# RIKEN-RCCS/EigenExa

Hardware: AMD Instinct MI355X
Metric: eigen_sx full-solve throughput (reference flop model: 4/3 N^3 + D&C GEMM + 2 nvec N^2) (higher is better)
Workload: dtype f64; 1 GPU; N=8192 random symmetric fp64 (counter-based R+R^T, seed 20240807), eigen_sx all eigenpairs, m_forward=64, m_backward=128; parallelism=1 GPU (1x1 grid)

## Files before the change

eigenexa_amd/csrc/api.hip:

```cpp
#include "eigx_context.h"
#include "eigx_comm.h"
#include "../../include/eigenexa_amd.h"
#include <cstring>

namespace eigx {
Context g_ctx;
}

using namespace eigx;

extern "C" {

int eigx_init(int device) {
  return eigx_init_multi(device, 0, 1, nullptr, 'C');
}

int eigx_get_device_count(void) {
  int ndev = 0;
  if (hipGetDeviceCount(&ndev) != hipSuccess) { (void)hipGetLastError(); return 0; }
  return ndev;
}

int eigx_get_rccl_unique_id(void* out128) {
  return comm_get_unique_id(out128);
// ... 15 lines not shown
  int ndev = 0;
  if (hipGetDeviceCount(&ndev) != hipSuccess || ndev <= 0) {
    fprintf(stderr, "[eigx] no HIP device visible: this library has no CPU path\n");
    return EIGX_ERR_NO_DEVICE;
  }
  if (device < 0 || device >= ndev) return EIGX_ERR_BAD_ARG;
  EIGX_HIP_CHECK(hipSetDevice(device));
  g_ctx.device = device;
  int Px = 1;
  for (int x = 1; x * x <= nranks; ++x)
    if (nranks % x == 0) Px = x;
  int req_px = 0, req_py = 0;
  if (g_next_px > 0) {
    const int rx = g_next_px, ry = g_next_py;
    req_px = rx; req_py = ry;
    g_next_px = g_next_py = 0;
    if (rx * ry != nranks) {
      fprintf(stderr, "[eigx] illegal grid dimensions %d x %d for %d ranks\n", rx, ry, nranks);
      return EIGX_ERR_BAD_ARG;
    }
    Px = rx;
  }
  Grid g;
  g.Px = Px;
  g.Py = nranks / Px;
  g.rank = rank;
  g.nranks = nranks;
  if (order == 'R' || order == 'r') {
    g.px = rank / g.Py;
    g.py = rank % g.Py;
    g.row_major = 1;
  } else {
    g.px = rank % g.Px;
    g.py = rank / g.Px;
    g.row_major = 0;
  }
  g_ctx.grid = g;
  if (nranks > 1) {
    const int rc = comm_init(g_ctx, uid);
    if (rc != 0) {
      g_ctx.grid = Grid();
      g_next_px = req_px; g_next_py = req_py;
      return rc;
    }
  }
  EIGX_HIP_CHECK(hipStreamCreateWithFlags(&g_ctx.stream, hipStreamNonBlocking));
  EIGX_HIP_CHECK(hipStreamCreateWithFlags(&g_ctx.side_stream, hipStreamNonBlocking));
  for (int q = 0; q < Context::kAux; ++q)
    EIGX_HIP_CHECK(hipStreamCreateWithFlags(&g_ctx.aux[q], hipStreamNonBlocking));
  for (int q = 0; q <= Context::kAux; ++q)
    EIGX_HIP_CHECK(hipEventCreateWithFlags(&g_ctx.aux_ev[q], hipEventDisableTiming));
  EIGX_HIP_CHECK(hipEventCreateWithFlags(&g_ctx.bt_ev, hipEventDisableTiming));
  EIGX_HIP_CHECK(hipEventCreateWithFlags(&g_ctx.dc_ev, hipEventDisableTiming));
  {
    int prio_lo = 0, prio_hi = 0;
    EIGX_HIP_CHECK(hipDeviceGetStreamPriorityRange(&prio_lo, &prio_hi));
    EIGX_HIP_CHECK(hipStreamCreateWithPriority(&g_ctx.dc_stream, hipStreamNonBlocking, prio_hi));
  }
  EIGX_HIP_CHECK(hipEventCreateWithFlags(&g_ctx.dc_b_ev, hipEventDisableTiming));
  EIGX_HIP_CHECK(hipEventCreateWithFlags(&g_ctx.dc_z_ev, hipEventDisableTiming));
  g_ctx.bt_stream = g_ctx.side_stream;
  g_ctx.initialized = true;
  g_ctx.errinfo = 0;
  return EIGX_OK;
}

int eigx_free(void) {
  if (!g_ctx.initialized) return EIGX_OK;
  EIGX_HIP_CHECK(hipSetDevice(g_ctx.device));
  EIGX_HIP_CHECK(hipDeviceSynchronize());
  if (g_ctx.grid.nranks > 1) comm_free(g_ctx);
  g_ctx.pool.release();
  for (hipEvent_t e : g_ctx.prof_ev) EIGX_HIP_CHECK(hipEventDestroy(e));
  EIGX_HIP_CHECK(hipStreamDestroy(g_ctx.stream));
  EIGX_HIP_CHECK(hipStreamDestroy(g_ctx.side_stream));
  for (int q = 0; q < Context::kAux; ++q) EIGX_HIP_CHECK(hipStreamDestroy(g_ctx.aux[q]));
  for (int q = 0; q <= Context::kAux; ++q) EIGX_HIP_CHECK(hipEventDestroy(g_ctx.aux_ev[q]));
  EIGX_HIP_CHECK(hipEventDestroy(g_ctx.bt_ev));
  EIGX_HIP_CHECK(hipEventDestroy(g_ctx.dc_ev));
  EIGX_HIP_CHECK(hipStreamDestroy(g_ctx.dc_stream));
  g_ctx.bt_stream = nullptr;
  EIGX_HIP_CHECK(hipEventDestroy(g_ctx.dc_b_ev));
  EIGX_HIP_CHECK(hipEventDestroy(g_ctx.dc_z_ev));
  g_ctx = Context();
  return EIGX_OK;
}

int eigx_get_version(int* version, char* date32, char* vcode32) {
  if (version) *version = 10;
  if (date32) { memset(date32, 0, 32); strncpy(date32, "2026-10", 31); }
  if (vcode32) { memset(vcode32, 0, 32); strncpy(vcode32, "eigenexa_amd gfx950", 31); }
  return EIGX_OK;
}

int eigx_get_procs(int* procs, int* x_procs, int* y_procs) {
  if (!g_ctx.initialized) return EIGX_ERR_NOT_INITIALIZED;
  if (procs) *procs = g_ctx.grid.nranks;
  if (x_procs) *x_procs = g_ctx.grid.Px;
  if (y_procs) *y_procs = g_ctx.grid.Py;
  return EIGX_OK;
}

int eigx_get_id(int* id, int* x_id, int* y_id) {
  if (!g_ctx.initialized) return EIGX_ERR_NOT_INITIALIZED;
  if (id) *id = g_ctx.grid.rank + 1;
  if (x_id) *x_id = g_ctx.grid.px + 1;
  if (y_id) *y_id = g_ctx.grid.py + 1;
  return EIGX_OK;
}

int eigx_get_comm(int* x_color, int* x_key, int* y_color, int* y_key) {
  if (!g_ctx.initialized) return EIGX_ERR_NOT_INITIALIZED;
  const Grid& g = g_ctx.grid;
  if (x_color) *x_color = g.py + 1;
  if (x_key) *x_key = g.px + 1;
  if (y_color) *y_color = g.px + 1;
  if (y_key) *y_key = g.py + 1;
  return EIGX_OK;
}

double eigx_comm_seconds(void) { return g_ctx.timers[4]; }

int eigx_comm_info(char* buf, int len) {
  if (!g_ctx.initialized) return EIGX_ERR_NOT_INITIALIZED;
  return comm_info(g_ctx, buf, len);
}

int eigx_get_errinfo(int64_t* info) {
  if (info) *info = g_ctx.errinfo;
  return EIGX_OK;
}

// ... 128 lines not shown
    out[3 * k + 1] += g_ctx.prof_units[q];
    out[3 * k + 2] += 1e-3 * ms;
  }
  return EIGX_OK;
}

int eigx_device_synchronize(void) {
  if (!g_ctx.initialized) return EIGX_ERR_NOT_INITIALIZED;
  EIGX_HIP_CHECK(hipSetDevice(g_ctx.device));
  EIGX_HIP_CHECK(hipDeviceSynchronize());
  return EIGX_OK;
}

void* eigx_malloc_dev(int64_t bytes) {
  if (!g_ctx.initialized) return nullptr;
  void* p = nullptr;
  if (hipMalloc(&p, (size_t)bytes) != hipSuccess) return nullptr;
  return p;
}
int eigx_free_dev(void* p) {
  if (p) EIGX_HIP_CHECK(hipFree(p));
  return EIGX_OK;
}
int eigx_memcpy_h2d(void* dst, const void* src, int64_t bytes) {
  EIGX_HIP_CHECK(hipMemcpy(dst, src, (size_t)bytes, hipMemcpyHostToDevice));
  return EIGX_OK;
}
int eigx_memcpy_d2h(void* dst, const void* src, int64_t bytes) {
  EIGX_HIP_CHECK(hipMemcpy(dst, src, (size_t)bytes, hipMemcpyDeviceToHost));
  return EIGX_OK;
}

int eigx_tune(int key, int value) {
  if (key == 0) return set_gemm_variant(value);
  if (key == 1) return set_bisect_threads(value);
  if (key == 2) return set_bt_q(value);
  if (key == 3 || key == 4 || key == 5 || key == 10 || key == 11) return set_reduce_knob(key, value);
  if (key == 12) return (value >= 0 && value <= 2) ? set_reduce_knob(key, value) : -1;
  if (key == 6) return set_gemm_cstream(value);
  if (key == 7) return value > 0 ? set_reduce_knob(key, value) : -1;
  if (key == 8) return set_dc_chunk(value);
  if (key == 9) return comm_set_bounce(value);
  if (key == 15) return set_dc_pipe(value);
  if (key == 16) return set_dc_batch(value);
  if (key == 17 || key == 18 || key == 19) return set_range_knob(key, value);
  if (key == 20) return set_tri_nb(value);
  if (key == 21) return set_batch_nmax(value);
  if (key == 22) return set_hbatch_nmax(value);
  if (key == 23) return set_gbatch_nmax(value);
  if (key == 24) return set_hgbatch_nmax(value);
  if (key == 25) return set_gemm_latec_kmax(value);
  if (key == 26) return set_batch_range_route(value);
  if (key == 27) return set_batch_range_accept(value);
  return -1;
}

int eigx_dgemm_dev(char opa, char opb, int m, int n, int k, double alpha, const double* a, int lda,
                   const double* b, int ldb, double beta, double* c, int ldc, int tri_upper) {
  if (!g_ctx.initialized) return EIGX_ERR_NOT_INITIALIZED;
  EIGX_HIP_CHECK(hipStreamSynchronize(nullptr));
  dgemm_dev(g_ctx.stream, opa, opb, m, n, k, alpha, a, lda, b, ldb, beta, c, ldc, tri_upper ? 1 : 0,
            &g_ctx.grid);
  EIGX_HIP_CHECK(hipStreamSynchronize(g_ctx.stream));
  return EIGX_OK;
}

int eigx_dgemm_gather_dev(char opa, char opb, int m, int n, int k, double alpha, const double* a, int lda,
                          const double* b, int ldb, double beta, double* c, int ldc, const int* kmap_a,
                          const int* kmap_b) {
  if (!g_ctx.initialized) return EIGX_ERR_NOT_INITIALIZED;
  EIGX_HIP_CHECK(hipStreamSynchronize(nullptr));
  dgemm_dev(g_ctx.stream, opa, opb, m, n, k, alpha, a, lda, b, ldb, beta, c, ldc, 0, nullptr, kmap_a, nullptr, 1, 0,
            0, 0, 1, 0, 0, 0, 1, 0, kmap_b);
  EIGX_HIP_CHECK(hipStreamSynchronize(g_ctx.stream));
  return EIGX_OK;
}

}
```

eigenexa_amd/csrc/band_reduce.hip:

```cpp
#include "eigx_context.h"
#include "eigx_comm.h"
#include "../../include/eigenexa_amd.h"
#include <algorithm>
#include <chrono>
#include <cstring>
#include <type_traits>

#pragma clang fp contract(on)

namespace eigx {

namespace {

static inline int pd_rows_for(int toprows) { int r = ((toprows + 3) / 4 + 63) / 64 * 64; return r < 512 ? 512 : r; }
#ifdef EIGX_STAMPS
#define EIGX_ABL(bit) (R.abl & (bit))
#define EIGX_STAMP(slot) do { if (R.dbg && threadIdx.x == 0 && stamp_me) { \
  const unsigned long long _t = __builtin_amdgcn_s_memtime(); atomicAdd(&R.dbg[slot], _t - stamp_prev); stamp_prev = _t; } } while (0)
#define EIGX_STAMP_INIT const bool stamp_me = (bid == nblocks / 2); unsigned long long stamp_prev = __builtin_amdgcn_s_memtime(); (void)stamp_me;
#else
#define EIGX_ABL(bit) false
#define EIGX_STAMP(slot) do {} while (0)
#define EIGX_STAMP_INIT
#endif
constexpr int PD_COLS = 16;
constexpr int KA_ROWS = 16;
constexpr int KA_SL = 256 / KA_ROWS;

enum { SC_SA = 0, SC_BETA_A = 1, SC_SB = 2, SC_BETA_B = 3, SC_COUNT = 8 };

struct RedArgs {
  double* A; int lda; int n;
  double* UW; int ldp; int m;
  double* X;
  double* YR; double* YC;
  double* KD;
  double* SP;
  int sp_packed;
  int kd_compact;
  double* GP;
  double* sc;
  double* d; double* e; int lde;
  int maxseg, maxrs, maxchunk, gp2_off, kdab_off;
  int P, me;
  float invP;
  int Px, Py, px, py, row_major;
  int nxs, nys;
  const double* MSG;
  int msg_stride;
  size_t ypar_stride; int ysrc_stride;
  const double* XW;
  int xmsg_stride, nown;
  size_t xpar_stride;
  const double* PAN; int ldpan;
  const double* zero16;
  int abl;
  int stamp_i;
  unsigned long long* dbg;
};

struct SymvGeom { int L, T, nt; };

int g_ka_fit = 1;
int g_ka_loads = 2;
int g_ka_wgs = 256;
int g_symv_t128 = 4500, g_symv_t256 = 40000;
int g_symv_nt = 9000;
int g_symv_unc = 9000;
}

int set_reduce_knob(int key, int v) {
  int* t = key == 3 ? &g_symv_t128 : key == 4 ? &g_symv_t256 : key == 5 ? &g_symv_nt : key == 7 ? &g_ka_wgs
         : key == 10 ? &g_ka_fit : key == 11 ? &g_symv_unc : key == 12 ? &g_ka_loads : nullptr;
  if (!t) return -1;
  const int old = *t;
  *t = v;
  return old;
}

namespace {

inline SymvGeom symv_geom(int L) {
  SymvGeom g;
  g.L = L;
  g.T = (L <= g_symv_t128) ? 128 : (L <= g_symv_t256 ? 256 : 512);
  g.nt = (L + g.T - 1) / g.T;
  return g;
}

typedef double d2v_t __attribute__((ext_vector_type(2)));
template <bool NT>
__device__ __forceinline__ double2 ld2(const double* p) {
  const d2v_t v = NT ? __builtin_nontemporal_load(reinterpret_cast<const d2v_t*>(p)) : *reinterpret_cast<const d2v_t*>(p);
  return make_double2(v.x, v.y);
}

template <int CTRL>
__device__ __forceinline__ double dpp_add(double v) {
  const int lo = __double2loint(v), hi = __double2hiint(v);
  const int lo2 = __builtin_amdgcn_update_dpp(0, lo, CTRL, 0xf, 0xf, true);
  const int hi2 = __builtin_amdgcn_update_dpp(0, hi, CTRL, 0xf, 0xf, true);
  return v + __hiloint2double(hi2, lo2);
}

template <int CTRL>
__device__ __forceinline__ double dpp_mov(double v) {
  const int lo2 = __builtin_amdgcn_update_dpp(0, __double2loint(v), CTRL, 0xf, 0xf, true);
  const int hi2 = __builtin_amdgcn_update_dpp(0, __double2hiint(v), CTRL, 0xf, 0xf, true);
  return __hiloint2double(hi2, lo2);
}

__device__ __forceinline__ double swapadd32(double a, double b) {
  const auto lo = __builtin_amdgcn_permlane32_swap(__double2loint(a), __double2loint(b), false, false);
  const auto hi = __builtin_amdgcn_permlane32_swap(__double2hiint(a), __double2hiint(b), false, false);
  return __hiloint2double(hi[0], lo[0]) + __hiloint2double(hi[1], lo[1]);
}
__device__ __forceinline__ double swapadd16(double a, double b) {
  const auto lo = __builtin_amdgcn_permlane16_swap(__double2loint(a), __double2loint(b), false, false);
  const auto hi = __builtin_amdgcn_permlane16_swap(__double2hiint(a), __double2hiint(b), false, false);
  return __hiloint2double(hi[0], lo[0]) + __hiloint2double(hi[1], lo[1]);
}

__device__ __forceinline__ double wave_sum(double v) {
  v = dpp_add<0xB1>(v);
  v = dpp_add<0x4E>(v);
  v = dpp_add<0x141>(v);
  v = dpp_add<0x140>(v);
// ... 1464 lines not shown
__global__ void compact_panel_kernel(const double* __restrict__ UW, int ldp, int m, int nrl, int ncl, int Px, int px,
                                     int Py, int py, double* __restrict__ UWr, int ldr, double* __restrict__ UWc, int ldc) {
  const int k = blockIdx.y;
  const double* rsrc = UW + (size_t)k * ldp;
  const double* csrc = UW + (size_t)(k + m) * ldp;
  for (int l = blockIdx.x * blockDim.x + threadIdx.x; l < (nrl > ncl ? nrl : ncl); l += gridDim.x * blockDim.x) {
    if (l < nrl) UWr[(size_t)k * ldr + l] = rsrc[(size_t)l * Px + px];
    if (l < ncl) UWc[(size_t)k * ldc + l] = csrc[(size_t)l * Py + py];
  }
}

__global__ void pack_panel_kernel(const double* __restrict__ A, int lda, int lj0, int mloc, int nrl, int nxs,
                                  double* __restrict__ send) {
  const int ljr = blockIdx.y;
  if (ljr >= mloc) return;
  for (int li = blockIdx.x * blockDim.x + threadIdx.x; li < nrl; li += gridDim.x * blockDim.x)
    send[(size_t)ljr * nxs + li] = A[(size_t)(lj0 + ljr) * lda + li];
}
__global__ void unpack_panel_kernel(const double* __restrict__ recv, size_t count, int nxs, int clo, int chi, int toprows,
                                    int Px, int Py, int row_major, double* __restrict__ PAN, int ldpan) {
  const int c = clo + blockIdx.y;
  if (c > chi) return;
  const int qy = c % Py;
  const int lj0 = (clo - qy + Py - 1) / Py;
  const int ljr = c / Py - lj0;
  for (int r = blockIdx.x * blockDim.x + threadIdx.x; r < toprows; r += gridDim.x * blockDim.x) {
    const int qx = r % Px;
    const int src = row_major ? qx * Py + qy : qx + qy * Px;
    PAN[(size_t)(c - clo) * ldpan + r] = ld_sys(recv + (size_t)src * count + (size_t)ljr * nxs + r / Px);
  }
}

template <int NB>
__global__ void mg_wcopy_kernel(RedArgs R, int xpar, int wk, int rows, StepWait W) {
  if (W.n > 0) step_wait_fused(W, blockIdx.x == 0);
  double* Wp = R.UW + (size_t)R.ldp * R.m;
  for (int r = blockIdx.x * blockDim.x + threadIdx.x; r < rows; r += gridDim.x * blockDim.x) {
    int s_, o_;
    own_of(R, r, s_, o_);
    const double* xm = R.XW + (size_t)xpar * R.xpar_stride + (size_t)s_ * R.xmsg_stride + o_;
    Wp[(size_t)wk * R.ldp + r] = ld_sys(xm + 2 * (size_t)R.nown);
    if (NB == 2) Wp[(size_t)(wk + 1) * R.ldp + r] = ld_sys(xm + 3 * (size_t)R.nown);
  }
}
template <int NB>
__global__ void mg_tail_kernel(RedArgs R, int xpar, int i, int ncols, StepWait W) {
  if (W.n > 0) step_wait_fused(W, blockIdx.x == 0);
  if (threadIdx.x == 0 && ncols > 0) {
    R.d[i] = xget<true>(R, xpar, 0, i);
    if (ncols > 1) { R.e[i] = xget<true>(R, xpar, 0, i - 1); R.d[i - 1] = xget<true>(R, xpar, 1, i - 1); }
  }
}

inline double wall_seconds() { return std::chrono::duration<double>(std::chrono::steady_clock::now().time_since_epoch()).count(); }
inline StepWait no_wait() { return StepWait{nullptr, nullptr, nullptr, 0, 0, 0, 1}; }
inline void clear_panel(const RedArgs& R, hipStream_t st) {
  hipLaunchKernelGGL(fill_kernel, dim3(1024), dim3(256), 0, st, R.UW, (size_t)R.ldp * R.m * 3, 0.0);
}

template <int NB>
RedArgs reduce_setup(Context& ctx, int n, double* A, int lda, double* d, double* e, int lde, int m) {
  m = std::min(std::max(m, NB), 256);
  if (NB == 2 && (m & 1)) ++m;
  const int ldp = pad_ld((n + 127) / 128 * 128 + 128);
  const Grid& G = ctx.grid;
  const bool mg = G.nranks > 1;
  RedArgs R;
  R.A = A; R.lda = lda; R.n = n; R.ldp = ldp; R.m = m;
  R.d = d; R.e = e; R.lde = lde;
  R.P = G.nranks; R.me = G.rank; R.invP = 1.0f / (float)G.nranks;
  R.Px = G.Px; R.Py = G.Py; R.px = G.px; R.py = G.py; R.row_major = G.row_major;
  R.nxs = (ceil_div(n, G.Px) + 7) / 8 * 8; R.nys = (ceil_div(n, G.Py) + 7) / 8 * 8;
  R.msg_stride = NB * (R.nxs + R.nys) + 8 + 2 * NB * m;
  R.ypar_stride = (size_t)G.nranks * R.msg_stride; R.ysrc_stride = R.msg_stride;
  R.nown = ceil_div(ceil_div(n, KA_ROWS), G.nranks) * KA_ROWS;
  R.xmsg_stride = 4 * R.nown + 8;
  R.xpar_stride = (size_t)G.nranks * R.xmsg_stride;
  R.MSG = nullptr; R.XW = nullptr; R.PAN = nullptr; R.ldpan = ldp;
  int maxseg = 0;
  if (mg) maxseg = ceil_div(R.nxs > R.nys ? R.nxs : R.nys, 128) + 1;
  else for (int L = n; L >= 1; --L) maxseg = std::max(maxseg, symv_geom(L).nt);
  maxseg += 1;
  R.maxseg = maxseg; R.maxrs = maxseg; R.maxchunk = 4 + 1;
  R.UW = ctx.pool.get_t<double>("red.UW", (size_t)ldp * (m * 3 + 128));
  R.X = ctx.pool.get_t<double>("red.X", (size_t)ldp * 3);
  if (!mg) {
    const int nslot = (maxseg + 2 > 162) ? maxseg + 2 : 162;
    R.YC = ctx.pool.get_t<double>("red.Y", (size_t)nslot * NB * ldp);
    R.YR = R.YC + (size_t)NB * ldp;
    R.kdab_off = R.maxchunk * 2 * NB * m;
    R.KD = ctx.pool.get_t<double>("red.KD", (size_t)R.kdab_off + R.maxchunk + 8 + 512);
  } else {
    R.YR = ctx.pool.get_t<double>("red.YR", (size_t)maxseg * NB * ldp);
    R.YC = ctx.pool.get_t<double>("red.YC", (size_t)R.maxrs * NB * ldp);
    const int maxchunk2 = 12;
    R.kdab_off = maxchunk2 * 2 * NB * m;
    R.KD = ctx.pool.get_t<double>("red.KD2", (size_t)R.kdab_off + 4 * G.nranks + 4 + 8 + 512);
  }
  R.SP = ctx.pool.get_t<double>("red.SP", (size_t)(maxseg * maxseg) * 3 + 8);
  R.sp_packed = (!mg && g_ka_loads >= 1) ? 1 : 0;
  R.kd_compact = (!mg && g_ka_loads >= 2) ? 1 : 0;
  R.gp2_off = 0;
  R.GP = ctx.pool.get_t<double>("red.GP", (size_t)((n + KA_ROWS - 1) / KA_ROWS + 2) * 3 + 8);
  R.sc = ctx.pool.get_t<double>("red.sc", SC_COUNT + 8);
  R.zero16 = R.sc + SC_COUNT;
  R.dbg = nullptr; R.abl = 0; R.stamp_i = -1;
#ifdef EIGX_STAMPS
  R.abl = getenv("EIGX_ABL") ? atoi(getenv("EIGX_ABL")) : 0;
  R.stamp_i = getenv("EIGX_STAMP_I") ? atoi(getenv("EIGX_STAMP_I")) : -1;
  R.dbg = ctx.pool.get_t<unsigned long long>("red.dbg", 4096);
  EIGX_HIP_CHECK(hipMemsetAsync(R.dbg, 0, 4096 * sizeof(unsigned long long), ctx.stream));
#endif
  clear_panel(R, ctx.stream);
  hipLaunchKernelGGL(fill_kernel, dim3(8), dim3(256), 0, ctx.stream, e, (size_t)lde * NB, 0.0);
  hipLaunchKernelGGL(fill_kernel, dim3(1), dim3(64), 0, ctx.stream, R.sc, (size_t)SC_COUNT + 8, 0.0);
  hipLaunchKernelGGL(fill_kernel, dim3(16), dim3(256), 0, ctx.stream, R.SP, (size_t)(maxseg * maxseg) * 3 + 8, 0.0);
  return R;
}

struct RedCounters {
  long n_symv = 0, n_k1 = 0; double symv_bytes = 0.0, k1_flops = 0.0;
  bool sampled(const Context& ctx) const { return ctx.prof_stride > 0 && (n_symv % ctx.prof_stride) == 0; }
  void step(int L) { symv_bytes += 8.0 * ((double)L * (L + 1) / 2); ++n_symv; }
  void panel(int nr, int m) { k1_flops += 2.0 * (double)nr * nr * m; ++n_k1; }
  void write(Context& ctx) const { ctx.timers[6] = (double)n_k1; ctx.timers[7] = k1_flops; ctx.timers[9] = (double)n_symv; ctx.timers[10] = symv_bytes; }
};
inline KAArgs ka_first_args() { KAArgs S{}; S.lgT_prev = 7; S.G = 1; S.wait = no_wait(); return S; }
template <int NB>
inline int ka_step_args(KAArgs& S, int i, int k) {
  const int L = i - NB + 1;
  S.ncols = (L >= 1) ? NB : (i >= 0 ? (i + 1 < NB ? i + 1 : NB) : 0);
  S.i = i; S.L = (L >= 1) ? L : 0; S.k = k;
  S.rows = (S.has_prev && S.iprev + 1 > i + 1) ? S.iprev + 1 : i + 1;
  return L;
}
template <int NB>
inline void step_done(KAArgs& S, RedCounters& C, int& i, int& k, int L, int nt, int T, int nchunk, int nchunk_ab) {
  C.step(L);
  S.has_prev = 1; S.iprev = i; S.Lprev = L; S.kprev = k; S.nchunk_prev = nchunk; S.nchunk_ab = nchunk_ab;
  S.nt_prev = nt; S.lgT_prev = (T == 128) ? 7 : (T == 256 ? 8 : 9);
  k += NB;
  i -= NB;
}
template <int NB>
inline bool panel_full(int k, int m, int i) { return k >= m && i - NB + 1 >= 1; }
inline void panel_restart(const RedArgs& R, RedCounters& C, KAArgs& S, int& k, int nr, hipStream_t st) {
  C.panel(nr, R.m); clear_panel(R, st); S.has_prev = 0; k = 0;
}
inline KAArgs ka_close_args(const KAArgs& S, int i, int k) { KAArgs F = S; F.ncols = 0; F.i = i; F.L = 0; F.k = k; F.rows = S.iprev + 1; return F; }
inline KBArgs kb_step_args(int i, int L, int k) {
  KBArgs B;
  B.i = i; B.L = L; B.k = k;
  B.ncg = (k + PD_COLS - 1) / PD_COLS; B.toprows = i + 1; B.pdr = pd_rows_for(B.toprows);
  B.nown_L = 0; B.npd_s = 0; B.pdr_s = 0; B.wk = -1; B.xpar = 0; B.xwait = no_wait();
  B.Lr = L; B.Lc = L; B.ntc = 0; B.nty_last = 0; B.slope = 0; B.c1 = 0;
  return B;
}
inline void trace_enqueue(double t_begin, hipStream_t st) {
  if (!getenv("EIGX_TRACE_ENQUEUE")) return;
  const double te = wall_seconds();
  EIGX_HIP_CHECK(hipStreamSynchronize(st));
  fprintf(stderr, "[eigx] reduction: enqueue loop %.1f ms, then %.1f ms until the stream drained\n", (te - t_begin) * 1e3, (wall_seconds() - te) * 1e3);
}
inline void stamps_report(const RedArgs& R, int NB, hipStream_t st) {
#ifdef EIGX_STAMPS
  const bool mg = R.P > 1;
// ... 49 lines not shown
    auto go_kb = [&](auto kb, auto pwc) {
      constexpr int RPB = decltype(rpb)::value, SPB = decltype(spb)::value, KB = decltype(kb)::value, PW = decltype(pwc)::value;
      constexpr bool SPK = decltype(spk)::value;
      if (K.G > 1) hipLaunchKernelGGL((ka_kernel<NB, false, true, RPB, SPB, KB, PW, SPK>), dim3(nwg), dim3(256), 0, st, R, K);
      else hipLaunchKernelGGL((ka_kernel<NB, false, false, RPB, SPB, KB, PW, SPK>), dim3(nwg), dim3(256), 0, st, R, K);
    };
    auto go_pw = [&](auto kb) {
      if constexpr (decltype(spk)::value) {
        if constexpr (decltype(kb)::value <= 4) {
          if (pw == 1) return go_kb(kb, IC<1>{});
        }
        if (pw == 2) return go_kb(kb, IC<2>{});
      }
      go_kb(kb, IC<0>{});
    };
    if (kk <= 2 * KA_SL) go_pw(IC<2>{}); else if (kk <= 4 * KA_SL) go_pw(IC<4>{}); else go_pw(IC<8>{});
  };
  if (R.sp_packed) {
    const std::true_type pk{};
    if (nslot <= 1 * KA_SL && ntl <= 256) go(IC<1>{}, IC<1>{}, pk);
    else if (nslot <= 2 * KA_SL && ntl <= 256) go(IC<2>{}, IC<1>{}, pk);
    else if (nslot <= 2 * KA_SL && ntl <= 512) go(IC<2>{}, IC<2>{}, pk);
    else if (nslot <= 3 * KA_SL && ntl <= 768) go(IC<3>{}, IC<3>{}, pk);
    else if (nslot <= 3 * KA_SL && ntl <= 1024) go(IC<3>{}, IC<4>{}, pk);
    else if (nslot <= 3 * KA_SL) go(IC<3>{}, IC<8>{}, pk);
    else if (nslot <= 5 * KA_SL) go(IC<5>{}, IC<8>{}, pk);
    else go(IC<10>{}, IC<8>{}, pk);
    return;
  }
  const std::false_type fl{};
  if (nslot <= 1 * KA_SL && ntp <= 15) go(IC<1>{}, IC<2>{}, fl);
  else if (nslot <= 2 * KA_SL && ntp <= 31) go(IC<2>{}, IC<4>{}, fl);
  else if (nslot <= 3 * KA_SL) go(IC<3>{}, IC<8>{}, fl);
  else if (nslot <= 5 * KA_SL) go(IC<5>{}, IC<8>{}, fl);
  else go(IC<10>{}, IC<8>{}, fl);
}

template <class Go>
void symv_variant(int T, bool nt_loads, bool unc, Go&& go) {
  auto u = [&](auto rb, auto ntl) { if (unc) go(rb, ntl, std::true_type{}); else go(rb, ntl, std::false_type{}); };
  if (T == 128) u(IC<1>{}, std::false_type{});
  else if (T == 256 && !nt_loads) u(IC<2>{}, std::false_type{});
  else if (T == 256) u(IC<2>{}, std::true_type{});
  else if (!nt_loads) u(IC<4>{}, std::false_type{});
  else u(IC<4>{}, std::true_type{});
}
template <int NB>
void launch_symv(hipStream_t st, int gx, const RedArgs& R, const KBArgs& B, int T, bool nt_loads, bool unc) {
  symv_variant(T, nt_loads, unc, [&](auto rb, auto ntl, auto un) {
    hipLaunchKernelGGL((symv_kernel<NB, decltype(rb)::value, decltype(ntl)::value, false, decltype(un)::value>), dim3(gx), dim3(256), 0, st, R, B);
  });
}

template <int NB>
void reduce_one_gpu(Context& ctx, const RedArgs& R, RedCounters& C) {
  const hipStream_t st = ctx.stream;
  const int m = R.m, ldp = R.ldp;
  const double t_begin = wall_seconds();
  KAArgs S = ka_first_args();
  int k = 0, i = R.n - 1;
  while (true) {
    const int L = ka_step_args<NB>(S, i, k);
    const int nb_ka = ka_grid_one_gpu(S.rows, S.G);
    if (S.rows > 0 && (S.has_prev || S.ncols > 0)) launch_ka<NB>(st, nb_ka, R, S);
    if (L < 1) break;
    KBArgs B = kb_step_args(i, L, k);
    const SymvGeom g = symv_geom(L);
    B.npd = (B.toprows + B.pdr - 1) / B.pdr; B.ngp = nb_ka; B.nt = g.nt; B.ng = g.T / 32;
    const int gx = g.nt * (g.nt + 1) / 2 + B.npd * (B.ncg + 1);
    const bool prof = C.sampled(ctx);
    if (prof) ctx.prof_begin(0, 8.0 * ((double)L * (L + 1) / 2), st);
    launch_symv<NB>(st, gx, R, B, g.T, L > g_symv_nt, L <= g_symv_unc);
    if (prof) ctx.prof_end(st);
    step_done<NB>(S, C, i, k, L, g.nt, g.T, B.npd, B.npd);
    if (panel_full<NB>(k, m, i)) {
      KAArgs F = ka_close_args(S, i, k);
      const int nb_kf = ka_grid_one_gpu(F.rows, F.G);
      launch_ka<NB>(st, nb_kf, R, F);
      const int nr = i + 1;
      if (ctx.prof_stride > 0) ctx.prof_begin(1, 2.0 * (double)nr * nr * m, st);
      dgemm_dev(st, 'N', 'T', nr, nr, 2 * m, -1.0, R.UW, ldp, R.UW + (size_t)ldp * m, ldp, 1.0, R.A, R.lda, 1);
      if (ctx.prof_stride > 0) ctx.prof_end(st);
      panel_restart(R, C, S, k, nr, st);
    }
  }
  trace_enqueue(t_begin, st);
}

template <int NB>
void launch_mg_step(hipStream_t st, int gx, const RedArgs& R, const KLArgs& KL, const KAArgs& S, const KBArgs& B,
                    const MGStep& M, int symv_T, bool nt_loads, bool unc) {
  if (symv_T == 0) hipLaunchKernelGGL((mg_step_kernel<NB, 1, false, true>), dim3(gx), dim3(256), 0, st, R, KL, S, B, M);
  else symv_variant(symv_T, nt_loads, unc, [&](auto rb, auto ntl, auto un) {
    hipLaunchKernelGGL((mg_step_kernel<NB, decltype(rb)::value, decltype(ntl)::value, decltype(un)::value>), dim3(gx), dim3(256), 0, st,
                       R, KL, S, B, M);
  });
}

inline int mg_step_geom(KBArgs& B, const Grid& G, int L, int& ntiles) {
  const int gfull = L / KA_ROWS, rem = L % KA_ROWS;
  B.nown_L = local_count(gfull, G.nranks, G.rank) * KA_ROWS + ((rem > 0 && gfull % G.nranks == G.rank) ? rem : 0);
  B.pdr = std::max(512, ((B.nown_L + 7) / 8 + 63) / 64 * 64);
  B.npd = (B.nown_L + B.pdr - 1) / B.pdr;
  B.pdr_s = std::max(512, ((B.toprows + 4 * G.nranks - 1) / (4 * G.nranks) + 63) / 64 * 64);
  B.npd_s = (B.toprows + B.pdr_s - 1) / B.pdr_s;
  B.ngp = G.nranks;
  B.Lr = local_count(L, G.Px, G.px); B.Lc = local_count(L, G.Py, G.py);
  const double leq = sqrt((double)(B.Lr > 1 ? B.Lr : 1) * (double)(B.Lc > 1 ? B.Lc : 1));
  const int T = (leq <= g_symv_t128) ? 128 : (leq <= g_symv_t256 ? 256 : 512);
  B.ntc = B.nt = ceil_div(B.Lc, T); B.ng = T / 32;
  ntiles = B.nty_last = B.ntc > 0 ? mg_nty(B.ntc - 1, T, B.Lc, G.Px, G.px, G.Py, G.py) : 0;
  for (int tx = 0; tx + 1 < B.ntc; ++tx) ntiles += mg_nty(tx, T, B.Lc, G.Px, G.px, G.Py, G.py);
  if (G.Py % G.Px == 0) { B.slope = G.Py / G.Px; B.c1 = (int)(((long)(T - 1) * G.Py + G.py - G.px) / ((long)G.Px * T)) + 1; }
  return T;
}

template <int NB>
void reduce_multi_rank(Context& ctx, RedArgs& R, RedCounters& C) {
  const hipStream_t st = ctx.stream;
  const Grid& G = ctx.grid;
  const int n = R.n, m = R.m, ldp = R.ldp;
  StepPeers peers, xpeers;
  R.MSG = comm_step_window(ctx, 0, (size_t)R.msg_stride, &peers); R.ysrc_stride = (int)peers.src_stride;
  R.XW = comm_step_window(ctx, 1, (size_t)R.xmsg_stride, &xpeers);
  unsigned long long epoch = comm_step_epoch_base(ctx, 0, (unsigned long long)(n / NB + 2));
  unsigned long long xepoch = comm_step_epoch_base(ctx, 1, (unsigned long long)(n / NB + n / m + 8));
  const int mloc_max = ceil_div(m + NB, G.Py) + 1;
  const size_t pan_count = (size_t)mloc_max * R.nxs;
  const int ldr = pad_ld(R.nxs + 2), ldc = pad_ld(R.nys + 2);
  PeerBuf* panr = comm_buffer(ctx, "red.panr", (size_t)G.nranks * pan_count * sizeof(double));
  double* pan = ctx.pool.get_t<double>("red.pan", (size_t)ldp * (m + NB));
  double* pan_send = ctx.pool.get_t<double>("red.pansend", pan_count);
  double* UWr = ctx.pool.get_t<double>("red.UWr", (size_t)ldr * 2 * m);
  double* UWc = ctx.pool.get_t<double>("red.UWc", (size_t)ldc * 2 * m);
  R.PAN = pan;
  EIGX_HIP_CHECK(hipMemsetAsync(pan_send, 0, pan_count * sizeof(double), st));
  auto panel_lo = [&](int itop) { const int clo = itop - m + 1; return clo <= NB ? 0 : clo; };
  auto gather_panel = [&](int clo, int chi, hipStream_t s, CommChannel ch) {
// ... 163 lines not shown
```

eigenexa_amd/csrc/eigx_context.h:

```cpp
#pragma once
#include "eigx_common.h"
#include <functional>
#include <map>
#include <vector>
#include <string>
#include <type_traits>

namespace eigx {

struct DeviceAllocError { size_t bytes; std::string name; };

struct Pool {
  struct Buf { void* p = nullptr; size_t bytes = 0; };
  std::map<std::string, Buf> bufs;
  void* get(const std::string& name, size_t bytes) {
    Buf& b = bufs[name];
    if (b.bytes < bytes) {
      if (b.p) EIGX_HIP_CHECK(hipFree(b.p));
      b.p = nullptr;
      b.bytes = 0;
      size_t want = bytes + bytes / 16 + 256;
      static const char* fail_name = getenv("EIGX_TEST_FAIL_ALLOC");
      if ((fail_name && name == fail_name) || hipMalloc(&b.p, want) != hipSuccess) {
        (void)hipGetLastError();
        b.p = nullptr;
        throw DeviceAllocError{want, name};
      }
      b.bytes = want;
    }
    return b.p;
  }
  template <typename T> T* get_t(const std::string& name, size_t count) {
    return (T*)get(name, count * sizeof(T));
  }
  std::map<std::string, Buf> hbufs;
  void* get_host(const std::string& name, size_t bytes) {
    Buf& b = hbufs[name];
    if (b.bytes < bytes) {
      if (b.p) EIGX_HIP_CHECK(hipHostFree(b.p));
      b.p = nullptr;
      size_t want = bytes + bytes / 16 + 256;
      EIGX_HIP_CHECK(hipHostMalloc(&b.p, want, hipHostMallocDefault));
      b.bytes = want;
    }
    return b.p;
  }
  void release() {
    for (auto& kv : bufs)
      if (kv.second.p) EIGX_HIP_CHECK(hipFree(kv.second.p));
    bufs.clear();
    for (auto& kv : hbufs)
      if (kv.second.p) EIGX_HIP_CHECK(hipHostFree(kv.second.p));
    hbufs.clear();
  }
};

struct CommState;

struct Context {
  bool initialized = false;
  int device = 0;
  Grid grid;
  hipStream_t stream = nullptr;
  hipStream_t side_stream = nullptr;
  static constexpr int kAux = 6;
  hipStream_t aux[kAux] = {nullptr, nullptr, nullptr, nullptr, nullptr, nullptr};
  hipEvent_t aux_ev[kAux + 1] = {nullptr, nullptr, nullptr, nullptr, nullptr, nullptr, nullptr};
  hipEvent_t bt_ev = nullptr;
  hipEvent_t dc_ev = nullptr;
  hipStream_t dc_stream = nullptr;
  hipStream_t bt_stream = nullptr;
  hipEvent_t dc_b_ev = nullptr, dc_z_ev = nullptr;
  int dc_zero_n = 0; const double* dc_zero_qa = nullptr; const double* dc_zero_qb = nullptr;
  bool bt_ready = false;
  const double* bt_a = nullptr; double* bt_V = nullptr;
  int bt_n = 0, bt_mb = 0, bt_band = 0, bt_ldv = 0;
  Pool pool;
  CommState* comm = nullptr;
  int64_t errinfo = 0;
  double timers[16] = {0};
  int prof_stride = 0;
  std::vector<hipEvent_t> prof_ev;
  std::vector<double> prof_units;
  std::vector<int> prof_kind;
  size_t prof_used = 0;
  void prof_begin(int kind, double units, hipStream_t st) {
    if (prof_used + 2 > prof_ev.size()) {
      for (int q = 0; q < 2; ++q) { hipEvent_t e; EIGX_HIP_CHECK(hipEventCreate(&e)); prof_ev.push_back(e); }
    }
    prof_kind.push_back(kind);
    prof_units.push_back(units);
    EIGX_HIP_CHECK(hipEventRecord(prof_ev[prof_used], st));
  }
  void prof_end(hipStream_t st) {
    EIGX_HIP_CHECK(hipEventRecord(prof_ev[prof_used + 1], st));
    prof_used += 2;
  }
};

extern Context g_ctx;

void comm_report_failure(Context& ctx, const char* what);

template <class F>
int eigx_guard(Context& ctx, F&& f) {
  try {
    return f();
  } catch (const DeviceAllocError& e) {
    fprintf(stderr, "[eigx] out of device memory: workspace '%s' needs %zu bytes\n", e.name.c_str(), e.bytes);
    comm_report_failure(ctx, "out of device memory on this rank");
    if (hipDeviceSynchronize() != hipSuccess) (void)hipGetLastError();
    return -8;
  }
}

int comm_get_unique_id(void* out128);
int comm_init(Context& ctx, const void* unique_id);
void comm_free(Context& ctx);

void band_reduce_dev(Context& ctx, int n, double* A, int lda, double* d, double* e, int lde, int m, int band);
// ... 202 lines not shown
```

Measured before the change: 19430 GFLOP/s.

## Finish small trailing reduction in one LDS-resident kernel; optional double-buffered panel clear

When the remaining matrix in the one-GPU blocked Householder reduction (NB=2) drops to a size that fits in LDS, the last panel is closed and one 1024-thread workgroup kernel does the rest. It keeps the packed triangle in shared memory and performs the two-column reflector, symv and rank-2 update per step. This replaces many small per-step launches and global-memory passes at the tail with a single launch, but runs on one compute unit. A second feature, off by default, double-buffers the UW panel buffer and clears the stale one on an aux stream, adding extra memory and event synchronisation.

```diff
diff --git a/eigenexa_amd/csrc/api.hip b/eigenexa_amd/csrc/api.hip
--- a/eigenexa_amd/csrc/api.hip
+++ b/eigenexa_amd/csrc/api.hip
@@ -91,6 +91,8 @@
     EIGX_HIP_CHECK(hipEventCreateWithFlags(&g_ctx.aux_ev[q], hipEventDisableTiming));
   EIGX_HIP_CHECK(hipEventCreateWithFlags(&g_ctx.bt_ev, hipEventDisableTiming));
   EIGX_HIP_CHECK(hipEventCreateWithFlags(&g_ctx.dc_ev, hipEventDisableTiming));
+  for (int q = 0; q < 4; ++q)
+    EIGX_HIP_CHECK(hipEventCreateWithFlags(&g_ctx.red_ev[q], hipEventDisableTiming | hipEventReleaseToDevice));
   {
     int prio_lo = 0, prio_hi = 0;
     EIGX_HIP_CHECK(hipDeviceGetStreamPriorityRange(&prio_lo, &prio_hi));
@@ -117,6 +119,7 @@
   for (int q = 0; q <= Context::kAux; ++q) EIGX_HIP_CHECK(hipEventDestroy(g_ctx.aux_ev[q]));
   EIGX_HIP_CHECK(hipEventDestroy(g_ctx.bt_ev));
   EIGX_HIP_CHECK(hipEventDestroy(g_ctx.dc_ev));
+  for (int q = 0; q < 4; ++q) EIGX_HIP_CHECK(hipEventDestroy(g_ctx.red_ev[q]));
   EIGX_HIP_CHECK(hipStreamDestroy(g_ctx.dc_stream));
   g_ctx.bt_stream = nullptr;
   EIGX_HIP_CHECK(hipEventDestroy(g_ctx.dc_b_ev));
@@ -351,6 +354,7 @@
   if (key == 25) return set_gemm_latec_kmax(value);
   if (key == 26) return set_batch_range_route(value);
   if (key == 27) return set_batch_range_accept(value);
+  if (key == 28 || key == 29) return set_reduce_knob(key, value);
   return -1;
 }
 
diff --git a/eigenexa_amd/csrc/band_reduce.hip b/eigenexa_amd/csrc/band_reduce.hip
--- a/eigenexa_amd/csrc/band_reduce.hip
+++ b/eigenexa_amd/csrc/band_reduce.hip
@@ -32,6 +32,7 @@
 struct RedArgs {
   double* A; int lda; int n;
   double* UW; int ldp; int m;
+  double* UW2;
   double* X;
   double* YR; double* YC;
   double* KD;
@@ -67,12 +68,28 @@
 int g_symv_t128 = 4500, g_symv_t256 = 40000;
 int g_symv_nt = 9000;
 int g_symv_unc = 9000;
+
+constexpr int TAIL_THREADS = 1024;
+constexpr int TAIL_ROWS = 256, TAIL_PARTS = TAIL_THREADS / TAIL_ROWS;
+constexpr size_t TAIL_LDS_BUDGET = 160 * 1024;
+constexpr size_t tail_lds_bytes(int L) { return 8 * ((size_t)L * (L + 1) / 2 + 2 * (size_t)TAIL_PARTS * L + 64); }
+constexpr int tail_max_size() {
+  int L = 0;
+  while (L + 1 <= TAIL_ROWS && tail_lds_bytes(L + 1) <= TAIL_LDS_BUDGET) ++L;
+  return L;
+}
+constexpr int TAIL_MAX = tail_max_size();
+int g_tail = TAIL_MAX;
+int g_panel_dbuf = 0;
 }
 
 int set_reduce_knob(int key, int v) {
   int* t = key == 3 ? &g_symv_t128 : key == 4 ? &g_symv_t256 : key == 5 ? &g_symv_nt : key == 7 ? &g_ka_wgs
-         : key == 10 ? &g_ka_fit : key == 11 ? &g_symv_unc : key == 12 ? &g_ka_loads : nullptr;
+         : key == 10 ? &g_ka_fit : key == 11 ? &g_symv_unc : key == 12 ? &g_ka_loads : key == 28 ? &g_tail
+         : key == 29 ? &g_panel_dbuf : nullptr;
   if (!t) return -1;
+  if (key == 28 && (v < 0 || v > TAIL_MAX)) return -1;
+  if (key == 29 && v != 0 && v != 1) return -1;
   const int old = *t;
   *t = v;
   return old;
@@ -1643,6 +1660,159 @@
   }
 }
 
+struct TailArgs { double* A; int lda; double* d; double* e; int lde; int n0; };
+
+__device__ __forceinline__ int tri_off(int c) { return c * (c + 1) / 2; }
+
+template <int K>
+__device__ __forceinline__ void tail_sum(double (&v)[K], double* red ) {
+  const int lane = threadIdx.x & 63, wave = threadIdx.x >> 6;
+#pragma unroll
+  for (int q = 0; q < K; ++q) v[q] = wave_sum(v[q]);
+  __syncthreads();
+  if (lane == 0 && wave < 4) {
+#pragma unroll
+    for (int q = 0; q < K; ++q) red[wave * K + q] = v[q];
+  }
+  __syncthreads();
+#pragma unroll
+  for (int q = 0; q < K; ++q) v[q] = (red[q] + red[K + q]) + (red[2 * K + q] + red[3 * K + q]);
+}
+
+__global__ __launch_bounds__(TAIL_THREADS) void tail_kernel(TailArgs Q) {
+  extern __shared__ __attribute__((aligned(16))) double tail_lds[];
+  const int n0 = Q.n0;
+  double2* pp = reinterpret_cast<double2*>(tail_lds);
+  double* red = tail_lds + 2 * TAIL_PARTS * n0;
+  double* tri = red + 64;
+  const int tid = threadIdx.x;
+  const int j = tid & (TAIL_ROWS - 1), s = tid / TAIL_ROWS;
+  const int jw = j & ~63;
+  const bool rowt = (s == 0);
+
+  const int tot = tri_off(n0);
+  for (int base = 0; base < tot; base += TAIL_THREADS * 8) {
+    double v[8];
+#pragma unroll
+    for (int q = 0; q < 8; ++q) {
+      const int idx = base + tid + TAIL_THREADS * q;
+      const int ic = (idx < tot) ? idx : 0;
+      int c = (int)((sqrtf(8.0f * (float)ic + 1.0f) - 1.0f) * 0.5f);
+      if (tri_off(c) > ic) --c;
+      if (tri_off(c + 1) <= ic) ++c;
+      v[q] = Q.A[(size_t)c * Q.lda + (ic - tri_off(c))];
+    }
+#pragma unroll
+    for (int q = 0; q < 8; ++q) {
+      const int idx = base + tid + TAIL_THREADS * q;
+      if (idx < tot) tri[idx] = v[q];
+    }
+  }
+  __syncthreads();
+
+  int i = n0 - 1;
+  for (; i - 1 >= 1; i -= 2) {
+    const int L = i - 1;
+    double* ci = tri + tri_off(i);
+    double* cm = tri + tri_off(i - 1);
+    const bool mine = rowt && j < L;
+    const double x0 = mine ? ci[j] : 0.0, x1 = mine ? cm[j] : 0.0;
+    const double x0L = ci[L - 1], x1L = cm[L - 1];
+    const double x0P = (L >= 2) ? ci[L - 2] : 0.0, x1P = (L >= 2) ? cm[L - 2] : 0.0;
+    const double dii = ci[i], eii = ci[i - 1], dmm = cm[i - 1];
+    double g[3] = {x0 * x0, x0 * x1, x1 * x1};
+    tail_sum<3>(g, red);
+    HouseScalars hs;
+    hs.sB = 0.0; hs.betaB = 0.0; hs.gammaB = 0.0;
+    if (g[0] > 0.0) { hs.sA = -sign_of(sqrt(g[0]), x0L); hs.betaA = g[0] - hs.sA * x0L; }
+    else { hs.sA = x0L; hs.betaA = 0.0; }
+    if (hs.betaA != 0.0) hs.gammaB = (g[1] - hs.sA * x1L) / hs.betaA;
+    hs.eL1 = x1L - hs.gammaB * (x0L - hs.sA);
+    double hB = g[2] - hs.eL1 * hs.eL1;
+    if (!(hB >= 0.25 * g[2])) {
+      const double t = x1 - hs.gammaB * x0;
+      double h[1] = {(mine && j < L - 1) ? t * t : 0.0};
+      tail_sum<1>(h, red);
+      hB = h[0];
+    }
+    {
+      const double xP = x1P - hs.gammaB * x0P;
+      if (hB > 0.0 && L >= 2) { hs.sB = -sign_of(sqrt(hB), xP); hs.betaB = hB - hs.sB * xP; }
+      else { hs.sB = (L >= 2) ? xP : 0.0; hs.betaB = 0.0; }
+    }
+    if (tid == 0) {
+      Q.d[i] = dii; Q.e[i] = eii; Q.d[i - 1] = dmm;
+      Q.e[Q.lde + i] = hs.sA;
+      Q.e[i - 1] = hs.eL1;
+      if (i - 1 >= 2) Q.e[Q.lde + i - 1] = hs.sB;
+    }
+    double uA = 0.0, uB = 0.0;
+    if (mine) {
+      uA = u_fix<2>(hs, L, 0, j, x0, x1);
+      uB = u_fix<2>(hs, L, 1, j, x0, x1);
+      ci[j] = uA; cm[j] = uB;
+      Q.A[(size_t)i * Q.lda + j] = uA;
+      Q.A[(size_t)(i - 1) * Q.lda + j] = uB;
+    }
+    __syncthreads();
+    if (j < L) {
+      const int tj = tri_off(j);
+      double pA = 0.0, pB = 0.0;
+#pragma unroll 4
+      for (int c = s; c < L; c += TAIL_PARTS) {
+        const double a = tri[(c <= j) ? tj + c : tri_off(c) + j];
+        pA += a * ci[c];
+        pB += a * cm[c];
+      }
+      pp[s * n0 + j] = make_double2(pA, pB);
+    }
+    __syncthreads();
+    double pA = 0.0, pB = 0.0;
+    double v[4] = {0.0, 0.0, 0.0, 0.0};
+    if (mine) {
+      const double2 q0 = pp[j], q1 = pp[n0 + j], q2 = pp[2 * n0 + j], q3 = pp[3 * n0 + j];
+      pA = ((q0.x + q1.x) + q2.x) + q3.x;
+      pB = ((q0.y + q1.y) + q2.y) + q3.y;
+      v[0] = uA * pA; v[1] = uA * pB; v[2] = uB * pB; v[3] = uA * uB;
+    }
+    tail_sum<4>(v, red);
+    {
+      const double tAA = (hs.betaA != 0.0) ? 1.0 / hs.betaA : 0.0;
+      const double tBB = (hs.betaB != 0.0) ? 1.0 / hs.betaB : 0.0;
+      const double gAA = v[0], gAB = v[1], gBB = v[2], uab = v[3];
+      const double tAB = -uab * tAA * tBB;
+      const double gt11 = gAA * tAA, gt12 = gAA * tAB + gAB * tBB;
+      const double gt21 = gAB * tAA, gt22 = gAB * tAB + gBB * tBB;
+      const double m11 = tAA * gt11, m12 = tAA * gt12;
+      const double m21 = tAB * gt11 + tBB * gt21, m22 = tAB * gt12 + tBB * gt22;
+      if (mine) {
+        const double yA = tAA * pA, yB = tAB * pA + tBB * pB;
+        const double wA = yA - 0.5 * (uA * m11 + uB * m21);
+        const double wB = yB - 0.5 * (uA * m12 + uB * m22);
+        pp[j] = make_double2(wA, wB);
+      }
+    }
+    __syncthreads();
+    if (j < L) {
+      const double uAj = ci[j], uBj = cm[j];
+      const double2 wj = pp[j];
+#pragma unroll 4
+      for (int c = jw + s; c < L; c += TAIL_PARTS) {
+        if (c >= j) {
+          const double2 wc = pp[c];
+          double* ap = tri + tri_off(c) + j;
+          *ap = *ap - ((uAj * wc.x + wj.x * ci[c]) + (uBj * wc.y + wj.y * cm[c]));
+        }
+      }
+    }
+    __syncthreads();
+  }
+  if (tid == 0) {
+    if (i == 1) { Q.d[1] = tri[2]; Q.e[1] = tri[1]; Q.d[0] = tri[0]; }
+    else if (i == 0) Q.d[0] = tri[0];
+  }
+}
+
 inline double wall_seconds() { return std::chrono::duration<double>(std::chrono::steady_clock::now().time_since_epoch()).count(); }
 inline StepWait no_wait() { return StepWait{nullptr, nullptr, nullptr, 0, 0, 0, 1}; }
 inline void clear_panel(const RedArgs& R, hipStream_t st) {
@@ -1675,7 +1845,9 @@
   R.maxseg = maxseg; R.maxrs = maxseg; R.maxchunk = 4 + 1;
   R.UW = ctx.pool.get_t<double>("red.UW", (size_t)ldp * (m * 3 + 128));
   R.X = ctx.pool.get_t<double>("red.X", (size_t)ldp * 3);
+  R.UW2 = nullptr;
   if (!mg) {
+    R.UW2 = ctx.pool.get_t<double>("red.UW2", (size_t)ldp * (m * 3 + 128));
     const int nslot = (maxseg + 2 > 162) ? maxseg + 2 : 162;
     R.YC = ctx.pool.get_t<double>("red.Y", (size_t)nslot * NB * ldp);
     R.YR = R.YC + (size_t)NB * ldp;
@@ -1703,6 +1875,7 @@
   EIGX_HIP_CHECK(hipMemsetAsync(R.dbg, 0, 4096 * sizeof(unsigned long long), ctx.stream));
 #endif
   clear_panel(R, ctx.stream);
+  if (R.UW2) hipLaunchKernelGGL(fill_kernel, dim3(1024), dim3(256), 0, ctx.stream, R.UW2, (size_t)R.ldp * R.m * 3, 0.0);
   hipLaunchKernelGGL(fill_kernel, dim3(8), dim3(256), 0, ctx.stream, e, (size_t)lde * NB, 0.0);
   hipLaunchKernelGGL(fill_kernel, dim3(1), dim3(64), 0, ctx.stream, R.sc, (size_t)SC_COUNT + 8, 0.0);
   hipLaunchKernelGGL(fill_kernel, dim3(16), dim3(256), 0, ctx.stream, R.SP, (size_t)(maxseg * maxseg) * 3 + 8, 0.0);
@@ -1858,11 +2031,33 @@
   });
 }
 
+inline void launch_tail(hipStream_t st, const RedArgs& R, int n0) {
+  static bool attr_set = false;
+  if (!attr_set) {
+    EIGX_HIP_CHECK(hipFuncSetAttribute((const void*)tail_kernel, hipFuncAttributeMaxDynamicSharedMemorySize, (int)tail_lds_bytes(TAIL_MAX)));
+    attr_set = true;
+  }
+  TailArgs Q{R.A, R.lda, R.d, R.e, R.lde, n0};
+  hipLaunchKernelGGL(tail_kernel, dim3(1), dim3(TAIL_THREADS), tail_lds_bytes(n0), st, Q);
+}
+
 template <int NB>
-void reduce_one_gpu(Context& ctx, const RedArgs& R, RedCounters& C) {
+void reduce_one_gpu(Context& ctx, const RedArgs& R0, RedCounters& C) {
   const hipStream_t st = ctx.stream;
+  RedArgs R = R0;
   const int m = R.m, ldp = R.ldp;
   const double t_begin = wall_seconds();
+  const int tail = (NB == 2) ? g_tail : 0;
+  if (tail > 0 && R.n <= tail) {
+    launch_tail(st, R, R.n);
+    trace_enqueue(t_begin, st);
+    return;
+  }
+  const bool dbuf = g_panel_dbuf != 0 && R.UW2 != nullptr;
+  const hipStream_t cs = ctx.aux[0];
+  double* const buf[2] = {R0.UW, R0.UW2};
+  bool clearing[2] = {false, false};
+  int cur = 0;
   KAArgs S = ka_first_args();
   int k = 0, i = R.n - 1;
   while (true) {
@@ -1879,17 +2074,39 @@
     launch_symv<NB>(st, gx, R, B, g.T, L > g_symv_nt, L <= g_symv_unc);
     if (prof) ctx.prof_end(st);
     step_done<NB>(S, C, i, k, L, g.nt, g.T, B.npd, B.npd);
-    if (panel_full<NB>(k, m, i)) {
+    const bool to_tail = tail > 0 && i + 1 <= tail;
+    if (panel_full<NB>(k, m, i) || to_tail) {
       KAArgs F = ka_close_args(S, i, k);
       const int nb_kf = ka_grid_one_gpu(F.rows, F.G);
       launch_ka<NB>(st, nb_kf, R, F);
       const int nr = i + 1;
-      if (ctx.prof_stride > 0) ctx.prof_begin(1, 2.0 * (double)nr * nr * m, st);
+      const bool prof1 = ctx.prof_stride > 0 && !to_tail;
+      if (prof1) ctx.prof_begin(1, 2.0 * (double)nr * nr * m, st);
       dgemm_dev(st, 'N', 'T', nr, nr, 2 * m, -1.0, R.UW, ldp, R.UW + (size_t)ldp * m, ldp, 1.0, R.A, R.lda, 1);
-      if (ctx.prof_stride > 0) ctx.prof_end(st);
-      panel_restart(R, C, S, k, nr, st);
-    }
-  }
+      if (prof1) ctx.prof_end(st);
+      if (!dbuf) {
+        panel_restart(R, C, S, k, nr, st);
+      } else {
+        C.panel(nr, m); S.has_prev = 0; k = 0;
+        EIGX_HIP_CHECK(hipEventRecord(ctx.red_ev[cur], st));
+        EIGX_HIP_CHECK(hipStreamWaitEvent(cs, ctx.red_ev[cur], 0));
+        RedArgs Rc = R;
+        Rc.UW = buf[cur];
+        clear_panel(Rc, cs);
+        EIGX_HIP_CHECK(hipEventRecord(ctx.red_ev[2 + cur], cs));
+        clearing[cur] = true;
+        cur ^= 1;
+        R.UW = buf[cur];
+        if (clearing[cur]) { EIGX_HIP_CHECK(hipStreamWaitEvent(st, ctx.red_ev[2 + cur], 0)); clearing[cur] = false; }
+      }
+    }
+    if (to_tail) {
+      launch_tail(st, R, i + 1);
+      break;
+    }
+  }
+  for (int b = 0; b < 2; ++b)
+    if (clearing[b]) EIGX_HIP_CHECK(hipStreamWaitEvent(st, ctx.red_ev[2 + b], 0));
   trace_enqueue(t_begin, st);
 }
 
diff --git a/eigenexa_amd/csrc/eigx_context.h b/eigenexa_amd/csrc/eigx_context.h
--- a/eigenexa_amd/csrc/eigx_context.h
+++ b/eigenexa_amd/csrc/eigx_context.h
@@ -66,6 +66,7 @@
   static constexpr int kAux = 6;
   hipStream_t aux[kAux] = {nullptr, nullptr, nullptr, nullptr, nullptr, nullptr};
   hipEvent_t aux_ev[kAux + 1] = {nullptr, nullptr, nullptr, nullptr, nullptr, nullptr, nullptr};
+  hipEvent_t red_ev[4] = {nullptr, nullptr, nullptr, nullptr};
   hipEvent_t bt_ev = nullptr;
   hipEvent_t dc_ev = nullptr;
   hipStream_t dc_stream = nullptr;
```

Result: no change. 19490 GFLOP/s (median of 5 runs) (+0.3%).
